# pyg-team/pyg-lib

Hardware: AMD Instinct MI355X
Metric: segment_matmul GFLOP/s + sampled-edges/sec, 1/2/4/8 MI355X vs CPU ref (higher is better)
Workload: dtype bf16; 1 GPU; segment_matmul ogbn-mag-shaped: 154 relations, 21,111,007 rows, F_in=F_out=128 (BASELINE.json configs[1]); relations=154, rows=21111007, rows_per_gpu=21111007, F=128

## Files before the change

### pyg_lib_amd/csrc/hip/matmul_dw.hip

```cpp
#include "matmul_dw_out.h"

#include <stdint.h>

#include <algorithm>
#include <atomic>

namespace pyg_hip {
namespace {

typedef __bf16 bf16x8 __attribute__((ext_vector_type(8)));
typedef _Float16 f16x8 __attribute__((ext_vector_type(8)));
typedef short v4i16 __attribute__((ext_vector_type(4)));
typedef short v8i16 __attribute__((ext_vector_type(8)));
typedef float f32x16 __attribute__((ext_vector_type(16)));
typedef uint32_t u32x4 __attribute__((ext_vector_type(4)));

constexpr int kTile = 128;

struct bf16_tag {};
struct f16_tag {};
template <typename Tag>
struct OutOf;
template <>
struct OutOf<bf16_tag> {
  using type = bf16_t;
};
template <>
struct OutOf<f16_tag> {
  using type = f16_t;
};

__device__ __forceinline__ f32x16 mfma16(bf16_tag, v8i16 a, v8i16 b, f32x16 c) {
  return __builtin_amdgcn_mfma_f32_32x32x16_bf16(__builtin_bit_cast(bf16x8, a), __builtin_bit_cast(bf16x8, b), c, 0, 0, 0);
}
__device__ __forceinline__ f32x16 mfma16(f16_tag, v8i16 a, v8i16 b, f32x16 c) {
  return __builtin_amdgcn_mfma_f32_32x32x16_f16(__builtin_bit_cast(f16x8, a), __builtin_bit_cast(f16x8, b), c, 0, 0, 0);
}

constexpr int pitch_bytes(int cols) {
  const int dw = cols / 2;
  const int extra = dw > 16 ? (dw - 16 + 63) / 64 : 0;
  return (16 + 64 * extra) * 4;
}

typedef const __attribute__((address_space(1))) u32x4 GU32x4;

template <typename Tag, int K, int MC>
__global__ __launch_bounds__(256, 1) void seg_dw_kernel(const DwGroup* __restrict__ groups,
                                                         const int32_t* __restrict__ tile_start, int B, int M,
                                                         float* __restrict__ slabs,
                                                         typename OutOf<Tag>::type* __restrict__ out) {
  constexpr int IB = K / 32, JB = MC / 32;
  constexpr int PX = pitch_bytes(K), PY = pitch_bytes(MC);
  constexpr int CX = K / 8, CY = MC / 8;
  constexpr int NX = 32 * CX / 64, NY = 32 * CY / 64;
  static_assert(IB * JB <= 16, "accumulators must fit the register file");
  extern __shared__ __attribute__((aligned(16))) char smem[];
  const int tid = threadIdx.x, lane = tid & 63, wave = tid >> 6;
  const int swave = __builtin_amdgcn_readfirstlane(wave);
  char* xs = smem + wave * 32 * (PX + PY);
  char* ys = xs + 32 * PX;
  const int ncol = M / MC;
  const int bx = ncol > 1 ? ((int)blockIdx.x / (8 * ncol)) * 8 + ((int)blockIdx.x & 7) : (int)blockIdx.x;
  const int by = ncol > 1 ? ((int)blockIdx.x / 8) % ncol : 0;
  const int col0 = by * MC;

  const int total = tile_start[B];
  const int G = (int)gridDim.x / ncol;
  const int t_beg = (int)((int64_t)bx * total / G);
  const int t_end = (int)((int64_t)(bx + 1) * total / G);
  if (t_beg >= t_end) return;
  int g = 0;
  {
    int lo = 0, hi = B;
    while (hi - lo > 1) {
      const int mid = (lo + hi) >> 1;
      if (tile_start[mid] <= t_beg) lo = mid; else hi = mid;
    }
    g = lo;
  }

  f32x16 acc[IB][JB];
#pragma unroll
  for (int i = 0; i < IB; ++i)
#pragma unroll
    for (int j = 0; j < JB; ++j)
#pragma unroll
      for (int r = 0; r < 16; ++r) acc[i][j][r] = 0.0f;
  int acc_g = -1;

  auto flush = [&]() {
    if (acc_g < 0) return;
    using Pos = DwPosRows<IB, JB>;
    const int u0 = tile_start[acc_g], u1 = tile_start[acc_g + 1];
    const bool head = u0 < t_beg, tail = !head && u1 > t_end;
    float* slab = dw_slab(slabs, (int64_t)IB * JB * kDwBlockFloats, ncol, bx, by, head ? 0 : 1);
    typename OutOf<Tag>::type* base = out + ((int64_t)acc_g * K) * M + col0;
    dw_combine_waves<IB, JB>(acc, smem, swave, lane, [&](int bt, int q, dwf4 s) __attribute__((always_inline)) {
      if (head || tail) dw_quarter_to_slab(slab, bt, q, s, lane);
      else dw_quarter_to_out<Pos>(base, M, K, MC, bt, q, s, lane);
    });
#pragma unroll
    for (int i = 0; i < IB; ++i)
#pragma unroll
      for (int j = 0; j < JB; ++j)
#pragma unroll
        for (int r = 0; r < 16; ++r) acc[i][j][r] = 0.0f;
  };

  u32x4 xr[NX], yr[NY];
  int n_g = g;
  DwGroup gd = groups[g];
  auto prefetch = [&](int t) {
    while (t >= tile_start[n_g + 1]) {
      ++n_g;
      gd = groups[n_g];
    }
    const int64_t row0 = (int64_t)(t - tile_start[n_g]) * kTile + wave * 32;
#pragma unroll
    for (int it = 0; it < NX; ++it) {
      const int p = it * 64 + lane;
      const int64_t row = row0 + p / CX;
      u32x4 v = {0u, 0u, 0u, 0u};
      if (row < gd.rows) v = *(GU32x4*)(gd.x + row * K + (p % CX) * 8);
      xr[it] = v;
    }
#pragma unroll
    for (int it = 0; it < NY; ++it) {
      const int p = it * 64 + lane;
      const int64_t row = row0 + p / CY;
      u32x4 v = {0u, 0u, 0u, 0u};
      if (row < gd.rows) v = *(GU32x4*)(gd.dy + row * M + col0 + (p % CY) * 8);
      yr[it] = v;
    }
  };

  const int q = lane & 15, half = (lane >> 4) & 1, kb = lane >> 5;
  const int a_off = (kb * 8 + (q >> 2)) * PX + (half * 16 + (q & 3) * 4) * 2;
  const int b_off = (kb * 8 + (q >> 2)) * PY + (half * 16 + (q & 3) * 4) * 2;
  typedef __attribute__((address_space(3))) v4i16* lds_v4;

  prefetch(t_beg);
  for (int t = t_beg; t < t_end; ++t) {
    const int cur_g = n_g;
    if (cur_g != acc_g) {
      flush();
      acc_g = cur_g;
    }
#pragma unroll
    for (int it = 0; it < NX; ++it) {
      const int p = it * 64 + lane;
      *reinterpret_cast<u32x4*>(xs + (p / CX) * PX + (p % CX) * 16) = xr[it];
    }
#pragma unroll
    for (int it = 0; it < NY; ++it) {
      const int p = it * 64 + lane;
      *reinterpret_cast<u32x4*>(ys + (p / CY) * PY + (p % CY) * 16) = yr[it];
    }
    __builtin_amdgcn_fence(__ATOMIC_RELEASE, "wavefront");
    __builtin_amdgcn_wave_barrier();
    if (t + 1 < t_end) prefetch(t + 1);
#pragma unroll
    for (int ks = 0; ks < 2; ++ks) {
      v8i16 af[IB], bf[JB];
#pragma unroll
      for (int i = 0; i < IB; ++i) {
        const char* p = xs + a_off + ks * 16 * PX + i * 64;
        const v4i16 lo = __builtin_amdgcn_ds_read_tr16_b64_v4i16((lds_v4)(p));
        const v4i16 hi = __builtin_amdgcn_ds_read_tr16_b64_v4i16((lds_v4)(p + 4 * PX));
        af[i] = __builtin_shufflevector(lo, hi, 0, 1, 2, 3, 4, 5, 6, 7);
      }
#pragma unroll
      for (int j = 0; j < JB; ++j) {
        const char* p = ys + b_off + ks * 16 * PY + j * 64;
        const v4i16 lo = __builtin_amdgcn_ds_read_tr16_b64_v4i16((lds_v4)(p));
        const v4i16 hi = __builtin_amdgcn_ds_read_tr16_b64_v4i16((lds_v4)(p + 4 * PY));
        bf[j] = __builtin_shufflevector(lo, hi, 0, 1, 2, 3, 4, 5, 6, 7);
      }
#pragma unroll
      for (int i = 0; i < IB; ++i)
#pragma unroll
        for (int j = 0; j < JB; ++j) acc[i][j] = mfma16(Tag{}, af[i], bf[j], acc[i][j]);
    }
    __builtin_amdgcn_wave_barrier();
  }
  flush();
}

template <typename Tag>
__global__ __launch_bounds__(256, 1) void seg_dw_wide256_kernel(const DwGroup* __restrict__ groups,
                                                                const int32_t* __restrict__ tile_start, int B, int M,
                                                                float* __restrict__ slabs,
                                                                typename OutOf<Tag>::type* __restrict__ out) {
  constexpr int K = 256, MC = 256, IB = K / 32, JB = 2;
  constexpr int PX = pitch_bytes(K), PY = pitch_bytes(MC);
  constexpr int CX = K / 8, CY = MC / 8;
  constexpr int NX = 32 * CX / 256, NY = 32 * CY / 256;
  constexpr int IMG = 32 * (PX + PY);
  extern __shared__ __attribute__((aligned(16))) char smem[];
  const int tid = threadIdx.x, lane = tid & 63, wave = tid >> 6;
  const int swave = __builtin_amdgcn_readfirstlane(wave);
  const int ncol = M / MC;
  const int bx = ncol > 1 ? ((int)blockIdx.x / (8 * ncol)) * 8 + ((int)blockIdx.x & 7) : (int)blockIdx.x;
  const int by = ncol > 1 ? ((int)blockIdx.x / 8) % ncol : 0;
  const int col0 = by * MC;

  const int total = tile_start[B];
  const int G = (int)gridDim.x / ncol;
  const int t_beg = (int)((int64_t)bx * total / G);
  const int t_end = (int)((int64_t)(bx + 1) * total / G);
  if (t_beg >= t_end) return;
  int g = 0;
  {
    int lo = 0, hi = B;
    while (hi - lo > 1) {
      const int mid = (lo + hi) >> 1;
      if (tile_start[mid] <= t_beg) lo = mid; else hi = mid;
    }
    g = lo;
  }

  f32x16 acc[IB][JB];
#pragma unroll
  for (int i = 0; i < IB; ++i)
#pragma unroll
    for (int j = 0; j < JB; ++j)
#pragma unroll
      for (int r = 0; r < 16; ++r) acc[i][j][r] = 0.0f;
  int acc_g = -1;
  auto flush = [&]() {
    if (acc_g < 0) return;
    const int u0 = tile_start[acc_g], u1 = tile_start[acc_g + 1];
    const bool head = u0 < t_beg, tail = !head && u1 > t_end;
    float* slab = dw_slab(slabs, (int64_t)DwPosWide::kBlocks * kDwBlockFloats, ncol, bx, by, head ? 0 : 1);
    typename OutOf<Tag>::type* base = out + ((int64_t)acc_g * K) * M + col0;
    char* stage = smem + 2 * IMG + wave * 16384 + lane * 16;
#pragma unroll
    for (int Q = 0; Q < 4; ++Q) {
#pragma unroll
      for (int L = 0; L < 4; ++L) {
        const int b = Q * 4 + L;
#pragma unroll
        for (int q = 0; q < 4; ++q) {
          const dwf4 v = {acc[b / JB][b % JB][4 * q], acc[b / JB][b % JB][4 * q + 1], acc[b / JB][b % JB][4 * q + 2],
                          acc[b / JB][b % JB][4 * q + 3]};
          *reinterpret_cast<dwf4*>(stage + (L * 4 + q) * 1024) = v;
        }
      }
      __builtin_amdgcn_fence(__ATOMIC_RELEASE, "wavefront");
      __builtin_amdgcn_wave_barrier();
#pragma unroll 1
      for (int it = 0; it < 16; ++it) {
        const dwf4 v = *reinterpret_cast<const dwf4*>(stage + it * 1024);
        const int bt = swave * 16 + Q * 4 + (it >> 2), q = it & 3;
        if (head || tail) dw_quarter_to_slab(slab, bt, q, v, lane);
        else dw_quarter_to_out<DwPosWide>(base, M, K, MC, bt, q, v, lane);
      }
      __builtin_amdgcn_wave_barrier();
    }
#pragma unroll
    for (int i = 0; i < IB; ++i)
#pragma unroll
      for (int j = 0; j < JB; ++j)
#pragma unroll
        for (int r = 0; r < 16; ++r) acc[i][j][r] = 0.0f;
  };

  const int s_beg = t_beg * 4, s_end = t_end * 4;
  u32x4 xr[NX], yr[NY];
  int n_g = g;
  DwGroup gd = groups[g];
  auto prefetch = [&](int sl) {
    const int t = sl >> 2;
    while (t >= tile_start[n_g + 1]) {
      ++n_g;
      gd = groups[n_g];
    }
    const int64_t row0 = (int64_t)(t - tile_start[n_g]) * kTile + (sl & 3) * 32;
#pragma unroll
    for (int it = 0; it < NX; ++it) {
      const int p = it * 256 + tid;
      const int64_t row = row0 + p / CX;
      u32x4 v = {0u, 0u, 0u, 0u};
      if (row < gd.rows) v = *(GU32x4*)(gd.x + row * K + (p % CX) * 8);
      xr[it] = v;
    }
#pragma unroll
    for (int it = 0; it < NY; ++it) {
      const int p = it * 256 + tid;
      const int64_t row = row0 + p / CY;
      u32x4 v = {0u, 0u, 0u, 0u};
      if (row < gd.rows) v = *(GU32x4*)(gd.dy + row * M + col0 + (p % CY) * 8);
      yr[it] = v;
    }
  };
  auto park = [&](int buf) {
    char* xs = smem + buf * IMG;
    char* ys = xs + 32 * PX;
#pragma unroll
    for (int it = 0; it < NX; ++it) {
      const int p = it * 256 + tid;
      *reinterpret_cast<u32x4*>(xs + (p / CX) * PX + (p % CX) * 16) = xr[it];
    }
#pragma unroll
    for (int it = 0; it < NY; ++it) {
      const int p = it * 256 + tid;
      *reinterpret_cast<u32x4*>(ys + (p / CY) * PY + (p % CY) * 16) = yr[it];
    }
  };

  const int q = lane & 15, half = (lane >> 4) & 1, kb = lane >> 5;
  const int a_off = (kb * 8 + (q >> 2)) * PX + (half * 16 + (q & 3) * 4) * 2;
  const int b_off = (kb * 8 + (q >> 2)) * PY + (half * 16 + (q & 3) * 4) * 2 + wave * 128;
  typedef __attribute__((address_space(3))) v4i16* lds_v4;

  prefetch(s_beg);
  int g_img[2];
  g_img[0] = n_g;
  park(0);
  g_img[1] = n_g;
  if (s_beg + 1 < s_end) prefetch(s_beg + 1);
  int g_regs = n_g;
  __syncthreads();

  for (int sl = s_beg; sl < s_end; ++sl) {
    const int cur = (sl - s_beg) & 1;
    if (sl + 1 < s_end) {
      park(cur ^ 1);
      g_img[cur ^ 1] = g_regs;
      if (sl + 2 < s_end) {
        prefetch(sl + 2);
        g_regs = n_g;
      }
    }
    const int cur_g = g_img[cur];
    if (cur_g != acc_g) {
      flush();
      acc_g = cur_g;
    }
    const char* xs = smem + cur * IMG;
    const char* ys = xs + 32 * PX;
#pragma unroll
    for (int ks = 0; ks < 2; ++ks) {
      v8i16 af[IB], bf[JB];
#pragma unroll
      for (int i = 0; i < IB; ++i) {
        const char* p = xs + a_off + ks * 16 * PX + i * 64;
        const v4i16 lo = __builtin_amdgcn_ds_read_tr16_b64_v4i16((lds_v4)(p));
        const v4i16 hi = __builtin_amdgcn_ds_read_tr16_b64_v4i16((lds_v4)(p + 4 * PX));
        af[i] = __builtin_shufflevector(lo, hi, 0, 1, 2, 3, 4, 5, 6, 7);
      }
#pragma unroll
      for (int j = 0; j < JB; ++j) {
        const char* p = ys + b_off + ks * 16 * PY + j * 64;
        const v4i16 lo = __builtin_amdgcn_ds_read_tr16_b64_v4i16((lds_v4)(p));
        const v4i16 hi = __builtin_amdgcn_ds_read_tr16_b64_v4i16((lds_v4)(p + 4 * PY));
        bf[j] = __builtin_shufflevector(lo, hi, 0, 1, 2, 3, 4, 5, 6, 7);
      }
#pragma unroll
      for (int i = 0; i < IB; ++i)
#pragma unroll
        for (int j = 0; j < JB; ++j) acc[i][j] = mfma16(Tag{}, af[i], bf[j], acc[i][j]);
    }
    __syncthreads();
  }
  flush();
}

template <int K, int MC>
__global__ __launch_bounds__(256, 1) void seg_dw_f32_kernel(const DwGroup* __restrict__ groups,
                                                             const int32_t* __restrict__ tile_start, int B, int M,
                                                             float* __restrict__ slabs, float* __restrict__ out) {
  constexpr int IB = K / 32, JB = MC / 32;
  static_assert(IB * JB <= 16, "accumulators must fit the register file");
  constexpr int VA = IB >= 4 ? 4 : IB, VB = JB >= 4 ? 4 : JB;
  extern __shared__ __attribute__((aligned(16))) char smem[];
  const int tid = threadIdx.x, lane = tid & 63, wave = tid >> 6;
  const int swave = __builtin_amdgcn_readfirstlane(wave);
  const int li = lane & 31, kk = lane >> 5;
  const int ncol = M / MC;
  const int bx = ncol > 1 ? ((int)blockIdx.x / (8 * ncol)) * 8 + ((int)blockIdx.x & 7) : (int)blockIdx.x;
  const int by = ncol > 1 ? ((int)blockIdx.x / 8) % ncol : 0;
  const int col0 = by * MC;
  const int total = tile_start[B];
  const int G = (int)gridDim.x / ncol;
  const int t_beg = (int)((int64_t)bx * total / G);
  const int t_end = (int)((int64_t)(bx + 1) * total / G);
  if (t_beg >= t_end) return;
  int g = 0;
  {
    int lo = 0, hi = B;
    while (hi - lo > 1) {
      const int mid = (lo + hi) >> 1;
      if (tile_start[mid] <= t_beg) lo = mid; else hi = mid;
    }
    g = lo;
  }
  f32x16 acc[IB][JB];
#pragma unroll
  for (int i = 0; i < IB; ++i)
#pragma unroll
    for (int j = 0; j < JB; ++j)
#pragma unroll
      for (int r = 0; r < 16; ++r) acc[i][j][r] = 0.0f;
  int acc_g = -1;
  auto flush = [&]() {
    if (acc_g < 0) return;
    using Pos = DwPosF32<IB, JB>;
    const int u0 = tile_start[acc_g], u1 = tile_start[acc_g + 1];
    const bool head = u0 < t_beg, tail = !head && u1 > t_end;
    float* slab = dw_slab(slabs, (int64_t)IB * JB * kDwBlockFloats, ncol, bx, by, head ? 0 : 1);
    float* base = out + ((int64_t)acc_g * K) * M + col0;
    dw_combine_waves<IB, JB>(acc, smem, swave, lane, [&](int bt, int q, dwf4 s) __attribute__((always_inline)) {
      if (head || tail) dw_quarter_to_slab(slab, bt, q, s, lane);
      else dw_quarter_to_out<Pos>(base, M, K, MC, bt, q, s, lane);
    });
#pragma unroll
    for (int i = 0; i < IB; ++i)
#pragma unroll
      for (int j = 0; j < JB; ++j)
#pragma unroll
        for (int r = 0; r < 16; ++r) acc[i][j][r] = 0.0f;
  };
  constexpr int D = 8;
  const int n_it = (t_end - t_beg) * 16;
  float pa[D][IB], pb[D][JB];
  int pg[D];
  int lg = g;
  DwGroup ld = groups[lg];
  auto request = [&](int it, float (&a)[IB], float (&b)[JB], int& grp) {
    const int t = t_beg + (it >> 4);
    while (t >= tile_start[lg + 1]) {
      ++lg;
      ld = groups[lg];
    }
    grp = lg;
    const float* xp = reinterpret_cast<const float*>(ld.x);
    const float* yp = reinterpret_cast<const float*>(ld.dy);
    const int64_t row = (int64_t)(t - tile_start[lg]) * kTile + wave * 32 + 2 * (it & 15) + kk;
    const bool ok = row < ld.rows;
#pragma unroll
    for (int h = 0; h < IB / VA; ++h) {
      typedef float vecA __attribute__((ext_vector_type(VA)));
      vecA v;
#pragma unroll
      for (int e = 0; e < VA; ++e) v[e] = 0.0f;
      if (ok) v = *(const __attribute__((address_space(1))) vecA*)(xp + row * K + 32 * VA * h + VA * li);
#pragma unroll
      for (int e = 0; e < VA; ++e) a[VA * h + e] = v[e];
    }
#pragma unroll
    for (int h = 0; h < JB / VB; ++h) {
      typedef float vecB __attribute__((ext_vector_type(VB)));
      vecB v;
#pragma unroll
      for (int e = 0; e < VB; ++e) v[e] = 0.0f;
      if (ok) v = *(const __attribute__((address_space(1))) vecB*)(yp + row * M + col0 + 32 * VB * h + VB * li);
#pragma unroll
      for (int e = 0; e < VB; ++e) b[VB * h + e] = v[e];
    }
  };
#pragma unroll
  for (int k = 0; k < D; ++k) request(k, pa[k], pb[k], pg[k]);
  static_assert(16 % D == 0, "a chunk of D steps must stay inside one tile");
  for (int it0 = 0; it0 < n_it; it0 += D) {
    if (pg[0] != acc_g) {
      flush();
      acc_g = pg[0];
    }
#pragma unroll
    for (int k = 0; k < D; ++k) {
#pragma unroll
      for (int i = 0; i < IB; ++i)
#pragma unroll
        for (int j = 0; j < JB; ++j) acc[i][j] = __builtin_amdgcn_mfma_f32_32x32x2f32(pa[k][i], pb[k][j], acc[i][j], 0, 0, 0);
      if (it0 + k + D < n_it) request(it0 + k + D, pa[k], pb[k], pg[k]);
    }
  }
  flush();
}

template <typename Pos, typename OutT>
__global__ __launch_bounds__(256) void seg_dw_fixup_kernel(const int32_t* __restrict__ tile_start, int B, int K, int M, int MC,
                                                          int G, int fix_blocks, const float* __restrict__ slabs,
                                                          OutT* __restrict__ out) {
  constexpr int NBT = Pos::kBlocks;
  const int lane = threadIdx.x & 63, wave = threadIdx.x >> 6;
  if ((int)blockIdx.x >= fix_blocks) {
    const int g = (int)blockIdx.x - fix_blocks;
    if (tile_start[g + 1] != tile_start[g]) return;
    OutT* base = out + (int64_t)g * K * M;
    for (int i = threadIdx.x; i < K * M; i += 256) dw_put(base + i, 0.0f);
    return;
  }
  const int ncol = M / MC;
  const int v = (int)blockIdx.x * 4 + wave;
  const int m = v / (4 * NBT), piece = v - m * (4 * NBT);
  const int bt = piece >> 2, q = piece & 3;
  const int bx = m / ncol, by = m - bx * ncol;
  const int total = tile_start[B];
  const int t_beg = (int)((int64_t)bx * total / G), t_end = (int)((int64_t)(bx + 1) * total / G);
  if (t_beg >= t_end) return;
  int lo = 0, hi = B;
  while (hi - lo > 1) {
    const int mid = (lo + hi) >> 1;
    if (tile_start[mid] <= t_end - 1) lo = mid; else hi = mid;
  }
  const int u0 = tile_start[lo], u1 = tile_start[lo + 1];
  if (!(u1 > t_end && u0 >= t_beg)) return;
  const dwf4 s = dw_chain_sum(slabs, (int64_t)NBT * kDwBlockFloats, ncol, bx, by, G, total, u1, bt, q, lane);
  dw_quarter_to_out<Pos>(out + (int64_t)lo * K * M + by * MC, M, K, MC, bt, q, s, lane);
}

__host__ __device__ inline int64_t dw_describe(DwGroup& d, const char* x, const char* dy, int64_t rows, int64_t, int64_t, int,
                                               int64_t, int, int) {
  d.x = reinterpret_cast<const uint16_t*>(x);
  d.dy = reinterpret_cast<const uint16_t*>(dy);
  d.rows = rows;
  return 1;
}
__host__ __device__ inline int64_t dw_describe(DwGenGroup& d, const char* x, const char* dy, int64_t rows, int64_t k, int64_t m,
                                               int elt, int64_t acc_off, int kb, int mb) {
  auto mn = [](int a, int b) { return a < b ? a : b; };
  d.x = x;
  d.dy = dy;
  d.rows = rows;
  d.acc_off = acc_off;
  d.k = (int32_t)k;
  d.m = (int32_t)m;
  d.lx = (int16_t)mn(gen_log2_align((uint64_t)x), gen_log2_align((uint64_t)(k * elt)));
  d.ly = (int16_t)mn(gen_log2_align((uint64_t)dy), gen_log2_align((uint64_t)(m * elt)));
  d.nkb = (int16_t)((k + kb - 1) / kb);
  d.nmb = (int16_t)((m + mb - 1) / mb);
  return (int64_t)d.nkb * d.nmb;
}

template <typename Desc>
__global__ void dw_plan_kernel(const int64_t* __restrict__ ptr, int64_t B, const char* X, const char* dY, int64_t K, int64_t M,
                               int elt, int kb, int mb, Desc* __restrict__ groups, int32_t* __restrict__ tile_start) {
  __shared__ int64_t part[256];
  const int tid = threadIdx.x;
  const int64_t per = (B + 255) / 256;
  const int64_t beg = min((int64_t)tid * per, B), end = min(beg + per, B);
  Desc d;
  const int64_t blocks = dw_describe(d, X, dY, 0, K, M, elt, 0, kb, mb);
  int64_t t = 0;
  for (int64_t b = beg; b < end; ++b) {
    const int64_t r = ptr[b + 1] - ptr[b];
    t += r > 0 ? (r + kTile - 1) / kTile * blocks : 0;
  }
  part[tid] = t;
  __syncthreads();
  if (tid == 0) {
    int64_t acc = 0;
    for (int i = 0; i < 256; ++i) {
      const int64_t v = part[i];
      part[i] = acc;
      acc += v;
    }
    tile_start[B] = (int32_t)acc;
  }
  __syncthreads();
  t = part[tid];
  for (int64_t b = beg; b < end; ++b) {
    tile_start[b] = (int32_t)t;
    const int64_t p0 = ptr[b];
    const int64_t r = ptr[b + 1] - p0;
    dw_describe(d, X + p0 * K * elt, dY + p0 * M * elt, r > 0 ? r : 0, K, M, elt, b * K * M, kb, mb);
    groups[b] = d;
    t += r > 0 ? (r + kTile - 1) / kTile * blocks : 0;
  }
}

enum class DwFamily {
  kUnsupported,
  kInvalid,
  kGen,
  kSeg,
  kWide256,
};
struct DwRoute {
  DwFamily family;
  int K = 0, MC = 0;
};

inline bool dw_dtype_ok(int dtype) { return dtype == PYG_F32 || dtype == PYG_BF16 || dtype == PYG_F16; }
inline int dw_elt(int dtype) { return dtype == PYG_F32 ? 4 : 2; }
inline DwRoute dw_gen_route(int dtype) { return {DwFamily::kGen, kDwGenKB, dw_gen_mb(dw_elt(dtype))}; }

DwRoute choose_dw_route(int dtype, int64_t K, int64_t M, bool uniform, unsigned misalign) {
  if (!dw_dtype_ok(dtype)) return {DwFamily::kUnsupported};
  if (misalign % dw_elt(dtype) != 0) return {DwFamily::kInvalid};
  if (!uniform || misalign % 16 != 0 || !((K == 64 || K == 128 || K == 256) && M > 0 && M % 64 == 0)) {
    if (K >= (1LL << 21) || M >= (1LL << 21) || K * M >= (1LL << 28)) return {DwFamily::kUnsupported};
    return dw_gen_route(dtype);
  }
  if (dtype != PYG_F32 && K == 256 && M % 256 == 0) return {DwFamily::kWide256, 256, 256};
  return {DwFamily::kSeg, (int)K, K == 256 || M % 128 != 0 ? 64 : 128};
}

inline unsigned dw_misalign(uintptr_t operands, const void* out, int elt) {
  return (unsigned)((operands & 15) | ((uintptr_t)out & (uintptr_t)(elt - 1)));
}

const char* dw_route_name(int dtype, DwRoute r) {
  thread_local char name[32];
  const char* t = dtype == PYG_BF16 ? "bf16" : dtype == PYG_F16 ? "f16" : "f32";
  switch (r.family) {
    case DwFamily::kUnsupported: return "unsupported";
    case DwFamily::kInvalid: return "invalid";
    case DwFamily::kGen: return "gen";
    case DwFamily::kSeg: snprintf(name, sizeof(name), "seg_%s_k%d_mc%d", t, r.K, r.MC); break;
    case DwFamily::kWide256: snprintf(name, sizeof(name), "wide256_%s", t); break;
  }
  return name;
}

int dw_route_check(const char* op, DwRoute r, int64_t K, int64_t M) {
  if (r.family == DwFamily::kInvalid) return fail(PYG_HIP_ERR_INVALID, "%s: operands must be element-aligned", op);
  if (r.family == DwFamily::kUnsupported)
    return fail(PYG_HIP_ERR_UNSUPPORTED, "%s: K x M = %lld x %lld is beyond the kernel's 32-bit offsets", op, (long long)K,
                (long long)M);
  if (r.family == DwFamily::kGen)
    PYG_HIP_REQUIRE((K + r.K - 1) / r.K < 32768 && (M + r.MC - 1) / r.MC < 32768, "%s: K / M too large", op);
  return PYG_HIP_OK;
}

inline int64_t dw_ncol(DwRoute r, int64_t M) { return r.family == DwFamily::kGen ? 1 : M / r.MC; }
inline int64_t dw_grid_x(int64_t tiles_upper, int64_t ncol) {
  int64_t gx = std::max<int64_t>(1, std::min<int64_t>(tiles_upper, device_info().num_cus / ncol));
  if (ncol > 1) gx = (gx + 7) / 8 * 8;
  return gx;
}
inline size_t dw_slab_bytes(DwRoute r, int64_t M) {
  const int64_t ncol = dw_ncol(r, M);
  return (size_t)(dw_grid_x(INT64_MAX, ncol) * ncol) * 2 * (size_t)r.K * (size_t)r.MC * sizeof(float);
}

struct DwWorkspace {
  int64_t* ptr_copy;
  void* descs;
  int32_t* tile_start;
  float* slabs;
  size_t plan_bytes;
  size_t bytes;
};

DwWorkspace carve_dw(void* ws, int64_t B, size_t desc_size, size_t slab_bytes) {
  DwWorkspace w;
  size_t off = 0;
  auto take = [&](size_t bytes, size_t align) {
    void* p = reinterpret_cast<void*>(reinterpret_cast<uintptr_t>(ws) + off);
    off += align_up(bytes, align);
    return p;
  };
  w.ptr_copy = static_cast<int64_t*>(take(sizeof(int64_t) * (size_t)(B + 1), 256));
  w.descs = take(desc_size * (size_t)std::max<int64_t>(B, 1), 256);
  w.tile_start = static_cast<int32_t*>(take(sizeof(int32_t) * (size_t)(B + 1), 256));
  w.plan_bytes = off - (size_t)(static_cast<char*>(w.descs) - static_cast<char*>(ws));
  w.slabs = static_cast<float*>(take(slab_bytes, 1));
  w.bytes = off;
  return w;
}
DwWorkspace carve_dw(void* ws, int64_t B, DwRoute r, int64_t M) {
  return carve_dw(ws, B, r.family == DwFamily::kGen ? sizeof(DwGenGroup) : sizeof(DwGroup), dw_slab_bytes(r, M));
}

size_t dw_workspace_bytes(int64_t B, int64_t K, int64_t M, bool uniform) {
  size_t need = 0;
  for (int dtype : {PYG_BF16, PYG_F32}) {
    need = std::max(need, carve_dw(nullptr, B, dw_gen_route(dtype), M).bytes);
    const DwRoute r = choose_dw_route(dtype, K, M, uniform, 0);
    if (r.family == DwFamily::kSeg || r.family == DwFamily::kWide256) need = std::max(need, carve_dw(nullptr, B, r, M).bytes);
  }
  return need;
}

struct DwLaunch {
  const DwGroup* groups;
  const int32_t* tile_start;
  int64_t B, M;
  int64_t gx;
  float* slabs;
  void* out;
  hipStream_t stream;
};

template <typename Pos, typename OutT>
int launch_fixup(const DwLaunch& a, int K, int MC, OutT* out) {
  const int64_t ncol = a.M / MC;
  const int64_t fix_blocks = a.gx * ncol * Pos::kBlocks;
  hipLaunchKernelGGL((seg_dw_fixup_kernel<Pos, OutT>), dim3((unsigned)(fix_blocks + a.B)), dim3(256), 0, a.stream, a.tile_start,
                     (int)a.B, K, (int)a.M, MC, (int)a.gx, (int)fix_blocks, a.slabs, out);
  PYG_HIP_CHECK(hipGetLastError());
  return PYG_HIP_OK;
}

template <typename Tag, int K, int MC>
int launch_dw(const DwLaunch& a) {
  using OutT = typename OutOf<Tag>::type;
  OutT* out = static_cast<OutT*>(a.out);
  constexpr int lds = 4 * 32 * (pitch_bytes(K) + pitch_bytes(MC));
  static_assert(lds >= (K / 32) * (MC / 32) * 4096, "the combine area must fit the row images");
  const void* kern = reinterpret_cast<const void*>(&seg_dw_kernel<Tag, K, MC>);
  if (int rc_ = ensure_dynamic_lds(kern, lds)) return rc_;
  hipLaunchKernelGGL((seg_dw_kernel<Tag, K, MC>), dim3((unsigned)(a.gx * (a.M / MC))), dim3(256), lds, a.stream, a.groups,
                     a.tile_start, (int)a.B, (int)a.M, a.slabs, out);
  PYG_HIP_CHECK(hipGetLastError());
  return launch_fixup<DwPosRows<K / 32, MC / 32>, OutT>(a, K, MC, out);
}

template <typename Tag>
int launch_dw_wide256(const DwLaunch& a) {
  using OutT = typename OutOf<Tag>::type;
  OutT* out = static_cast<OutT*>(a.out);
  constexpr int lds = 2 * 32 * (pitch_bytes(256) + pitch_bytes(256)) + 4 * 16384;
  const void* kern = reinterpret_cast<const void*>(&seg_dw_wide256_kernel<Tag>);
  if (int rc_ = ensure_dynamic_lds(kern, lds)) return rc_;
  hipLaunchKernelGGL((seg_dw_wide256_kernel<Tag>), dim3((unsigned)(a.gx * (a.M / 256))), dim3(256), lds, a.stream, a.groups,
                     a.tile_start, (int)a.B, (int)a.M, a.slabs, out);
  PYG_HIP_CHECK(hipGetLastError());
  return launch_fixup<DwPosWide, OutT>(a, 256, 256, out);
}

template <int K, int MC>
int launch_dw_f32(const DwLaunch& a) {
  float* out = static_cast<float*>(a.out);
  constexpr int lds = (K / 32) * (MC / 32) * 4096;
  const void* kern = reinterpret_cast<const void*>(&seg_dw_f32_kernel<K, MC>);
  if (int rc_ = ensure_dynamic_lds(kern, lds)) return rc_;
  hipLaunchKernelGGL((seg_dw_f32_kernel<K, MC>), dim3((unsigned)(a.gx * (a.M / MC))), dim3(256), lds, a.stream, a.groups,
                     a.tile_start, (int)a.B, (int)a.M, a.slabs, out);
  PYG_HIP_CHECK(hipGetLastError());
  return launch_fixup<DwPosF32<K / 32, MC / 32>, float>(a, K, MC, out);
}

template <int K, int MC>
int launch_seg(int dtype, const DwLaunch& a) {
  return dtype == PYG_F32 ? launch_dw_f32<K, MC>(a) : dtype == PYG_BF16 ? launch_dw<bf16_tag, K, MC>(a) : launch_dw<f16_tag, K, MC>(a);
}

int run_dw_route(DwRoute r, int dtype, const DwWorkspace& w, int64_t B, int64_t M, int64_t tiles_upper, void* out, int lg,
                 hipStream_t stream) {
  const int64_t gx = dw_grid_x(tiles_upper, dw_ncol(r, M));
  const DwLaunch a = {static_cast<const DwGroup*>(w.descs), w.tile_start, B, M, gx, w.slabs, out, stream};
  switch (r.family) {
    case DwFamily::kGen: return launch_dw_gen(dtype, w.descs, w.tile_start, (int)B, gx, w.slabs, out, lg, stream);
    case DwFamily::kWide256: return dtype == PYG_BF16 ? launch_dw_wide256<bf16_tag>(a) : launch_dw_wide256<f16_tag>(a);
    case DwFamily::kSeg:
      if (r.K == 128 && r.MC == 128) return launch_seg<128, 128>(dtype, a);
      if (r.K == 128 && r.MC == 64) return launch_seg<128, 64>(dtype, a);
      if (r.K == 64 && r.MC == 128) return launch_seg<64, 128>(dtype, a);
      if (r.K == 64 && r.MC == 64) return launch_seg<64, 64>(dtype, a);
      if (r.K == 256 && r.MC == 64) return launch_seg<256, 64>(dtype, a);
      break;
    default: break;
  }
  return fail(PYG_HIP_ERR_INVALID, "matmul_dw: unknown route");
}

std::atomic<int64_t> g_dw_fast{0}, g_dw_gen{0};
inline int dw_count(DwRoute r, int rc) {
  if (rc == PYG_HIP_OK) ++(r.family == DwFamily::kGen ? g_dw_gen : g_dw_fast);
  return rc;
}

template <typename Desc>
int dw_segment(DwRoute r, int dtype, const void* input, const int64_t* ptr, int ptr_on_device, const void* grad_out,
               void* grad_other, int64_t N, int64_t K, int64_t M, int64_t B, void* workspace, hipStream_t stream) {
  const int elt = dw_elt(dtype);
  const char* X = static_cast<const char*>(input);
  const char* dY = static_cast<const char*>(grad_out);
  Desc d;
  const int64_t tiles_upper = ((N + kTile - 1) / kTile + B) * dw_describe(d, X, dY, 0, K, M, elt, 0, r.K, r.MC);
  PYG_HIP_REQUIRE(tiles_upper < (1LL << 31), "segment_matmul_dw: too many tiles");
  const DwWorkspace w = carve_dw(workspace, B, r, M);
  const int64_t* dptr = ptr;
  if (!ptr_on_device) {
    if (int rc = stage_host_ptr("segment_matmul_dw", ptr, B, N, w.ptr_copy, stream)) return rc;
    dptr = w.ptr_copy;
  }
  hipLaunchKernelGGL(dw_plan_kernel<Desc>, dim3(1), dim3(256), 0, stream, dptr, B, X, dY, K, M, elt, r.K, r.MC,
                     static_cast<Desc*>(w.descs), w.tile_start);
  PYG_HIP_CHECK(hipGetLastError());
  const int lg = gen_log2_align((uint64_t)input | (uint64_t)(K * elt) | (uint64_t)grad_out | (uint64_t)(M * elt));
  return run_dw_route(r, dtype, w, B, M, tiles_upper, grad_other, lg, stream);
}

template <typename Desc>
int dw_grouped(DwRoute r, int dtype, const pyg_hip_group* host_groups, int64_t G, void* out_pool, void* workspace,
               hipStream_t stream) {
  const int elt = dw_elt(dtype);
  const DwWorkspace w = carve_dw(workspace, G, r, host_groups[0].m);
  void* staged = nullptr;
  int rc = pinned_stage().acquire(w.plan_bytes, &staged);
  if (rc != PYG_HIP_OK) return rc;
  Desc* hd = static_cast<Desc*>(staged);
  int32_t* ht = reinterpret_cast<int32_t*>(static_cast<char*>(staged) + (reinterpret_cast<char*>(w.tile_start) - static_cast<char*>(w.descs)));
  int64_t t = 0, off = 0;
  int lg = 4;
  for (int64_t i = 0; i < G; ++i) {
    const pyg_hip_group& g = host_groups[i];
    ht[i] = (int32_t)t;
    t += (g.rows + kTile - 1) / kTile * dw_describe(hd[i], static_cast<const char*>(g.input), static_cast<const char*>(g.other),
                                                    g.rows, g.k, g.m, elt, off, r.K, r.MC);
    PYG_HIP_REQUIRE(t < (1LL << 31), "grouped_matmul_dw: too many tiles");
    if (g.rows > 0 && g.k > 0 && g.m > 0)
      lg = std::min(lg, gen_log2_align((uint64_t)g.input | (uint64_t)(g.k * elt) | (uint64_t)g.other | (uint64_t)(g.m * elt)));
    off += (int64_t)g.k * g.m;
  }
  ht[G] = (int32_t)t;
  PYG_HIP_CHECK(hipMemcpyAsync(w.descs, staged, w.plan_bytes, hipMemcpyHostToDevice, stream));
  rc = pinned_stage().commit(stream);
  if (rc != PYG_HIP_OK) return rc;
  if (r.family != DwFamily::kGen) return run_dw_route(r, dtype, w, G, host_groups[0].m, t + 1, out_pool, lg, stream);
  if (off == 0) return PYG_HIP_OK;
  if (t == 0) {
    PYG_HIP_CHECK(hipMemsetAsync(out_pool, 0, (size_t)elt * (size_t)off, stream));
    return PYG_HIP_OK;
  }
  return run_dw_route(r, dtype, w, G, 0, t, out_pool, lg, stream);
}

}
}

using namespace pyg_hip;

extern "C" {

void pyg_hip_matmul_dw_counters(int64_t* specialised, int64_t* general) {
  if (specialised) *specialised = g_dw_fast.load();
  if (general) *general = g_dw_gen.load();
}

const char* pyg_hip_matmul_dw_route(int dtype, int64_t K, int64_t M, int uniform, unsigned misalign) {
  if (K < 0 || M < 0) return "invalid";
  return dw_route_name(dtype, choose_dw_route(dtype, K, M, uniform != 0, misalign));
}

size_t pyg_hip_segment_matmul_dw_workspace_size(int64_t B, int64_t K, int64_t M) {
  return dw_workspace_bytes(std::max<int64_t>(B, 0), std::max<int64_t>(K, 0), std::max<int64_t>(M, 0), true);
}

size_t pyg_hip_grouped_matmul_dw_workspace_size(const pyg_hip_group* groups, int64_t G) {
  if (G <= 0 || groups == nullptr) return dw_workspace_bytes(0, 0, 0, false);
  bool uniform = true;
  for (int64_t i = 0; i < G; ++i) uniform = uniform && groups[i].k == groups[0].k && groups[i].m == groups[0].m;
  return dw_workspace_bytes(G, std::max(groups[0].k, 0), std::max(groups[0].m, 0), uniform);
}

int pyg_hip_segment_matmul_dw(int dtype, const void* input, const int64_t* ptr, int ptr_on_device, const void* grad_out,
                              void* grad_other, int64_t N, int64_t K, int64_t M, int64_t B, void* workspace,
                              size_t workspace_bytes, void* stream_) {
  hipStream_t stream = static_cast<hipStream_t>(stream_);
  PYG_HIP_REQUIRE(N >= 0 && K >= 0 && M >= 0 && B >= 0, "segment_matmul_dw: negative size");
  if (B * K * M == 0) return PYG_HIP_OK;
  PYG_HIP_REQUIRE(ptr && grad_other && (N == 0 || (input && grad_out)), "segment_matmul_dw: NULL tensor");
  if (!dw_dtype_ok(dtype))
    return fail(PYG_HIP_ERR_UNSUPPORTED, "segment_matmul_dw: float32 / bfloat16 / float16 only (dtype %d)", dtype);
  const size_t need = pyg_hip_segment_matmul_dw_workspace_size(B, K, M);
  if (workspace == nullptr || workspace_bytes < need)
    return fail(PYG_HIP_ERR_WORKSPACE, "segment_matmul_dw: workspace of %zu bytes needed, got %zu", need, workspace_bytes);
  const unsigned misalign = dw_misalign((uintptr_t)input | (uintptr_t)grad_out, grad_other, dw_elt(dtype));
  const DwRoute r = choose_dw_route(dtype, K, M, true, misalign);
  if (int rc = dw_route_check("segment_matmul_dw", r, K, M)) return rc;
  return dw_count(r, r.family == DwFamily::kGen
                         ? dw_segment<DwGenGroup>(r, dtype, input, ptr, ptr_on_device, grad_out, grad_other, N, K, M, B, workspace, stream)
                         : dw_segment<DwGroup>(r, dtype, input, ptr, ptr_on_device, grad_out, grad_other, N, K, M, B, workspace, stream));
}

int pyg_hip_grouped_matmul_dw(int dtype, const pyg_hip_group* host_groups, int64_t G, void* out_pool, void* workspace,
                              size_t workspace_bytes, void* stream_) {
  hipStream_t stream = static_cast<hipStream_t>(stream_);
  PYG_HIP_REQUIRE(G >= 0 && G < (1LL << 31), "grouped_matmul_dw: bad group count");
  if (G == 0) return PYG_HIP_OK;
  PYG_HIP_REQUIRE(host_groups && out_pool, "grouped_matmul_dw: NULL argument");
  if (!dw_dtype_ok(dtype))
    return fail(PYG_HIP_ERR_UNSUPPORTED, "grouped_matmul_dw: float32 / bfloat16 / float16 only (dtype %d)", dtype);
  const int64_t K = host_groups[0].k, M = host_groups[0].m;
  bool uniform = true;
  uintptr_t operands = 0;
  for (int64_t i = 0; i < G; ++i) {
    const pyg_hip_group& g = host_groups[i];
    PYG_HIP_REQUIRE(g.rows >= 0 && g.k >= 0 && g.m >= 0, "grouped_matmul_dw: negative size in group %lld", (long long)i);
    PYG_HIP_REQUIRE(g.rows == 0 || g.k == 0 || g.m == 0 || (g.input && g.other), "grouped_matmul_dw: NULL tensor in group %lld",
                    (long long)i);
    uniform = uniform && g.k == K && g.m == M;
    operands |= (uintptr_t)g.input | (uintptr_t)g.other;
  }
  const size_t need = pyg_hip_grouped_matmul_dw_workspace_size(host_groups, G);
  if (workspace == nullptr || workspace_bytes < need)
    return fail(PYG_HIP_ERR_WORKSPACE, "grouped_matmul_dw: workspace of %zu bytes needed, got %zu", need, workspace_bytes);
  const unsigned misalign = dw_misalign(operands, out_pool, dw_elt(dtype));
  const DwRoute r = choose_dw_route(dtype, K, M, uniform, misalign);
  for (int64_t i = 0; i < G; ++i) {
    const int64_t k = host_groups[i].k, m = host_groups[i].m;
    if (int rc = dw_route_check("grouped_matmul_dw", choose_dw_route(dtype, k, m, uniform, misalign), k, m)) return rc;
  }
  return dw_count(r, r.family == DwFamily::kGen ? dw_grouped<DwGenGroup>(r, dtype, host_groups, G, out_pool, workspace, stream)
                                                : dw_grouped<DwGroup>(r, dtype, host_groups, G, out_pool, workspace, stream));
}

}
```

Baseline: 388,600 GFLOP/s.

## Add ring-buffered direct-to-LDS pipeline for 128x128 segment dW kernel

Adds a new dW kernel for K=MC=128 in which each wave keeps a 4-slot LDS ring. The ring is filled with global_load_lds_dwordx4 (direct global-to-LDS, non-temporal) using XOR-swizzled offsets, and vmcnt waits let three items load ahead of the MFMA work. This removes the register staging and the per-tile LDS store/barrier round trip of the old kernel. Partial tail rows go through a separate zero-padded path. The default launch path now routes 128x128 to the new kernel. An experiment macro also adds a load-only probe mode. The hand-written m0 and vmcnt asm is fragile and adds correctness risk.

```diff
diff --git a/pyg_lib_amd/csrc/hip/matmul_dw.hip b/pyg_lib_amd/csrc/hip/matmul_dw.hip
--- a/pyg_lib_amd/csrc/hip/matmul_dw.hip
+++ b/pyg_lib_amd/csrc/hip/matmul_dw.hip
@@ -16,6 +16,10 @@
 typedef uint32_t u32x4 __attribute__((ext_vector_type(4)));
 
 constexpr int kTile = 128;
+
+#ifndef PYG_HIP_DW_EXPERIMENTS
+#define PYG_HIP_DW_EXPERIMENTS 0
+#endif
 
 struct bf16_tag {};
 struct f16_tag {};
@@ -147,6 +151,14 @@
       flush();
       acc_g = cur_g;
     }
+#if PYG_HIP_DW_EXPERIMENTS == 2
+#pragma unroll
+    for (int it = 0; it < NX; ++it) asm volatile("" ::"v"(xr[it]));
+#pragma unroll
+    for (int it = 0; it < NY; ++it) asm volatile("" ::"v"(yr[it]));
+    if (t + 1 < t_end) prefetch(t + 1);
+    continue;
+#endif
 #pragma unroll
     for (int it = 0; it < NX; ++it) {
       const int p = it * 64 + lane;
@@ -183,6 +195,194 @@
         for (int j = 0; j < JB; ++j) acc[i][j] = mfma16(Tag{}, af[i], bf[j], acc[i][j]);
     }
     __builtin_amdgcn_wave_barrier();
+  }
+  flush();
+}
+
+template <typename Tag>
+__global__ __launch_bounds__(256, 1) void seg_dw_ring_kernel(const DwGroup* __restrict__ groups,
+                                                              const int32_t* __restrict__ tile_start, int B, int M,
+                                                              float* __restrict__ slabs,
+                                                              typename OutOf<Tag>::type* __restrict__ out) {
+  constexpr int K = 128, MC = 128, IB = K / 32, JB = MC / 32;
+  constexpr int kItem = 8192, kSlots = 4;
+  extern __shared__ __attribute__((aligned(16))) char smem[];
+  const int tid = threadIdx.x, lane = tid & 63;
+  const int swave = __builtin_amdgcn_readfirstlane(tid >> 6);
+  char* ring = smem + swave * (kSlots * kItem);
+  const int ncol = M / MC;
+  const int bx = ncol > 1 ? ((int)blockIdx.x / (8 * ncol)) * 8 + ((int)blockIdx.x & 7) : (int)blockIdx.x;
+  const int by = ncol > 1 ? ((int)blockIdx.x / 8) % ncol : 0;
+  const int col0 = by * MC;
+
+  const int total = tile_start[B];
+  const int G = (int)gridDim.x / ncol;
+  const int t_beg = (int)((int64_t)bx * total / G);
+  const int t_end = (int)((int64_t)(bx + 1) * total / G);
+  if (t_beg >= t_end) return;
+  int g = 0;
+  {
+    int lo = 0, hi = B;
+    while (hi - lo > 1) {
+      const int mid = (lo + hi) >> 1;
+      if (tile_start[mid] <= t_beg) lo = mid; else hi = mid;
+    }
+    g = lo;
+  }
+
+  f32x16 acc[IB][JB];
+#pragma unroll
+  for (int i = 0; i < IB; ++i)
+#pragma unroll
+    for (int j = 0; j < JB; ++j)
+#pragma unroll
+      for (int r = 0; r < 16; ++r) acc[i][j][r] = 0.0f;
+  int acc_g = -1;
+
+  auto flush = [&]() {
+    if (acc_g < 0) return;
+    using Pos = DwPosRows<IB, JB>;
+    const int u0 = tile_start[acc_g], u1 = tile_start[acc_g + 1];
+    const bool head = u0 < t_beg, tail = !head && u1 > t_end;
+    float* slab = dw_slab(slabs, (int64_t)IB * JB * kDwBlockFloats, ncol, bx, by, head ? 0 : 1);
+    typename OutOf<Tag>::type* base = out + ((int64_t)acc_g * K) * M + col0;
+    dw_combine_waves<IB, JB>(acc, smem, swave, lane, [&](int bt, int q, dwf4 s) __attribute__((always_inline)) {
+      if (head || tail) dw_quarter_to_slab(slab, bt, q, s, lane);
+      else dw_quarter_to_out<Pos>(base, M, K, MC, bt, q, s, lane);
+    });
+    asm volatile("s_waitcnt vmcnt(0)" ::: "memory");
+#pragma unroll
+    for (int i = 0; i < IB; ++i)
+#pragma unroll
+      for (int j = 0; j < JB; ++j)
+#pragma unroll
+        for (int r = 0; r < 16; ++r) acc[i][j][r] = 0.0f;
+  };
+
+  const int l4 = lane >> 4, cs = lane & 15;
+  const uint32_t src_chunk = (uint32_t)((cs ^ (l4 << 2)) * 16);
+  uint32_t ox[4], oy[4];
+#pragma unroll
+  for (int j = 0; j < 4; ++j) {
+    ox[j] = (uint32_t)((4 * j + l4) * (K * 2)) + src_chunk;
+    oy[j] = (uint32_t)(4 * j + l4) * (uint32_t)(M * 2) + (uint32_t)(col0 * 2) + src_chunk;
+  }
+  const int q = lane & 15, half = (lane >> 4) & 1, kb = lane >> 5, rho = q >> 2;
+  int rd[4];
+#pragma unroll
+  for (int i = 0; i < 4; ++i) rd[i] = (kb * 8 + rho) * 256 + ((i ^ rho) * 64) + half * 32 + (q & 3) * 8;
+  typedef __attribute__((address_space(3))) v4i16* lds_v4;
+
+  DwGroup gd = groups[g];
+  const uint32_t ring_lds = (uint32_t)(size_t)ring;
+  auto issue = [&](int64_t row, int slot) {
+    const char* xb = reinterpret_cast<const char*>(gd.x) + row * (K * 2);
+    const char* yb = reinterpret_cast<const char*>(gd.dy) + row * ((int64_t)M * 2);
+    const uint32_t lds = ring_lds + (uint32_t)(slot * kItem);
+    uint32_t sv;
+    asm volatile(
+        "s_waitcnt lgkmcnt(0)\n\t"
+        "s_nop 4\n\t"
+        "s_mov_b32 %[sv], m0\n\t"
+        "s_mov_b32 m0, %[lds]\n\t"
+        "s_nop 0\n\t"
+        "global_load_lds_dwordx4 %[x0], %[xb] nt\n\t"
+        "s_add_u32 m0, m0, 0x400\n\ts_nop 0\n\t"
+        "global_load_lds_dwordx4 %[x1], %[xb] nt\n\t"
+        "s_add_u32 m0, m0, 0x400\n\ts_nop 0\n\t"
+        "global_load_lds_dwordx4 %[x2], %[xb] nt\n\t"
+        "s_add_u32 m0, m0, 0x400\n\ts_nop 0\n\t"
+        "global_load_lds_dwordx4 %[x3], %[xb] nt\n\t"
+        "s_add_u32 m0, m0, 0x400\n\ts_nop 0\n\t"
+        "global_load_lds_dwordx4 %[y0], %[yb] nt\n\t"
+        "s_add_u32 m0, m0, 0x400\n\ts_nop 0\n\t"
+        "global_load_lds_dwordx4 %[y1], %[yb] nt\n\t"
+        "s_add_u32 m0, m0, 0x400\n\ts_nop 0\n\t"
+        "global_load_lds_dwordx4 %[y2], %[yb] nt\n\t"
+        "s_add_u32 m0, m0, 0x400\n\ts_nop 0\n\t"
+        "global_load_lds_dwordx4 %[y3], %[yb] nt\n\t"
+        "s_mov_b32 m0, %[sv]"
+        : [sv] "=&s"(sv)
+        : [lds] "s"(lds), [xb] "s"(xb), [yb] "s"(yb), [x0] "v"(ox[0]), [x1] "v"(ox[1]), [x2] "v"(ox[2]), [x3] "v"(ox[3]),
+          [y0] "v"(oy[0]), [y1] "v"(oy[1]), [y2] "v"(oy[2]), [y3] "v"(oy[3])
+        : "memory", "scc");
+  };
+  auto wait_item = [&](int younger) {
+    if (younger >= 3) asm volatile("s_waitcnt vmcnt(24)" ::: "memory");
+    else if (younger == 2) asm volatile("s_waitcnt vmcnt(16)" ::: "memory");
+    else if (younger == 1) asm volatile("s_waitcnt vmcnt(8)" ::: "memory");
+    else asm volatile("s_waitcnt vmcnt(0)" ::: "memory");
+  };
+  auto multiply = [&](int slot) {
+    const char* xs = ring + slot * kItem;
+    const char* ys = xs + kItem / 2;
+    v8i16 af[IB], bf[JB];
+#pragma unroll
+    for (int i = 0; i < IB; ++i) {
+      const char* p = xs + rd[i];
+      const v4i16 lo = __builtin_amdgcn_ds_read_tr16_b64_v4i16((lds_v4)(p));
+      const v4i16 hi = __builtin_amdgcn_ds_read_tr16_b64_v4i16((lds_v4)(p + 4 * 256));
+      af[i] = __builtin_shufflevector(lo, hi, 0, 1, 2, 3, 4, 5, 6, 7);
+    }
+#pragma unroll
+    for (int j = 0; j < JB; ++j) {
+      const char* p = ys + rd[j];
+      const v4i16 lo = __builtin_amdgcn_ds_read_tr16_b64_v4i16((lds_v4)(p));
+      const v4i16 hi = __builtin_amdgcn_ds_read_tr16_b64_v4i16((lds_v4)(p + 4 * 256));
+      bf[j] = __builtin_shufflevector(lo, hi, 0, 1, 2, 3, 4, 5, 6, 7);
+    }
+#pragma unroll
+    for (int i = 0; i < IB; ++i)
+#pragma unroll
+      for (int j = 0; j < JB; ++j) acc[i][j] = mfma16(Tag{}, af[i], bf[j], acc[i][j]);
+  };
+  auto park_partial = [&](int64_t row, int nrows, int slot) {
+    char* xs = ring + slot * kItem;
+    char* ys = xs + kItem / 2;
+    u32x4 xv[4], yv[4];
+#pragma unroll
+    for (int j = 0; j < 4; ++j) {
+      xv[j] = u32x4{0u, 0u, 0u, 0u};
+      yv[j] = u32x4{0u, 0u, 0u, 0u};
+      if (4 * j + l4 < nrows) {
+        xv[j] = *(GU32x4*)(reinterpret_cast<const char*>(gd.x) + row * (K * 2) + ox[j]);
+        yv[j] = *(GU32x4*)(reinterpret_cast<const char*>(gd.dy) + row * ((int64_t)M * 2) + oy[j]);
+      }
+    }
+#pragma unroll
+    for (int j = 0; j < 4; ++j) {
+      *reinterpret_cast<u32x4*>(xs + j * 1024 + lane * 16) = xv[j];
+      *reinterpret_cast<u32x4*>(ys + j * 1024 + lane * 16) = yv[j];
+    }
+    __builtin_amdgcn_fence(__ATOMIC_RELEASE, "wavefront");
+    __builtin_amdgcn_wave_barrier();
+  };
+
+  for (int t = t_beg; t < t_end;) {
+    while (t >= tile_start[g + 1]) ++g;
+    const int g_end = tile_start[g + 1];
+    const int t1 = g_end < t_end ? g_end : t_end;
+    flush();
+    acc_g = g;
+    gd = groups[g];
+    const int64_t row0 = (int64_t)(t - tile_start[g]) * kTile + swave * 32;
+    const int T = t1 - t;
+    const int64_t left = gd.rows - (row0 + (int64_t)(T - 1) * kTile);
+    const int nf = 2 * (T - 1) + (left >= 32 ? 2 : left >= 16 ? 1 : 0);
+    const int pr = left > 0 && left < 32 ? (int)(left & 15) : 0;
+    auto row_of = [&](int n) { return row0 + (int64_t)(n >> 1) * kTile + (n & 1) * 16; };
+    for (int n = 0; n < kSlots - 1 && n < nf; ++n) issue(row_of(n), n);
+    for (int n = 0; n < nf; ++n) {
+      if (n + kSlots - 1 < nf) issue(row_of(n + kSlots - 1), (n + kSlots - 1) & (kSlots - 1));
+      wait_item(nf - 1 - n);
+      multiply(n & (kSlots - 1));
+    }
+    if (pr) {
+      park_partial(row_of(nf), pr, nf & (kSlots - 1));
+      multiply(nf & (kSlots - 1));
+    }
+    __builtin_amdgcn_wave_barrier();
+    t = t1;
   }
   flush();
 }
@@ -696,18 +896,36 @@
   return PYG_HIP_OK;
 }
 
+template <typename Tag>
+int launch_dw_ring(const DwLaunch& a) {
+  using OutT = typename OutOf<Tag>::type;
+  OutT* out = static_cast<OutT*>(a.out);
+  constexpr int lds = 4 * 4 * 8192;
+  static_assert(lds >= 16 * 4096, "the combine area must fit the rings");
+  const void* kern = reinterpret_cast<const void*>(&seg_dw_ring_kernel<Tag>);
+  if (int rc_ = ensure_dynamic_lds(kern, lds)) return rc_;
+  hipLaunchKernelGGL((seg_dw_ring_kernel<Tag>), dim3((unsigned)(a.gx * (a.M / 128))), dim3(256), lds, a.stream, a.groups,
+                     a.tile_start, (int)a.B, (int)a.M, a.slabs, out);
+  PYG_HIP_CHECK(hipGetLastError());
+  return launch_fixup<DwPosRows<4, 4>, OutT>(a, 128, 128, out);
+}
+
 template <typename Tag, int K, int MC>
 int launch_dw(const DwLaunch& a) {
   using OutT = typename OutOf<Tag>::type;
   OutT* out = static_cast<OutT*>(a.out);
-  constexpr int lds = 4 * 32 * (pitch_bytes(K) + pitch_bytes(MC));
-  static_assert(lds >= (K / 32) * (MC / 32) * 4096, "the combine area must fit the row images");
-  const void* kern = reinterpret_cast<const void*>(&seg_dw_kernel<Tag, K, MC>);
-  if (int rc_ = ensure_dynamic_lds(kern, lds)) return rc_;
-  hipLaunchKernelGGL((seg_dw_kernel<Tag, K, MC>), dim3((unsigned)(a.gx * (a.M / MC))), dim3(256), lds, a.stream, a.groups,
-                     a.tile_start, (int)a.B, (int)a.M, a.slabs, out);
-  PYG_HIP_CHECK(hipGetLastError());
-  return launch_fixup<DwPosRows<K / 32, MC / 32>, OutT>(a, K, MC, out);
+  if constexpr (K == 128 && MC == 128 && PYG_HIP_DW_EXPERIMENTS == 0) {
+    return launch_dw_ring<Tag>(a);
+  } else {
+    constexpr int lds = 4 * 32 * (pitch_bytes(K) + pitch_bytes(MC));
+    static_assert(lds >= (K / 32) * (MC / 32) * 4096, "the combine area must fit the row images");
+    const void* kern = reinterpret_cast<const void*>(&seg_dw_kernel<Tag, K, MC>);
+    if (int rc_ = ensure_dynamic_lds(kern, lds)) return rc_;
+    hipLaunchKernelGGL((seg_dw_kernel<Tag, K, MC>), dim3((unsigned)(a.gx * (a.M / MC))), dim3(256), lds, a.stream, a.groups,
+                       a.tile_start, (int)a.B, (int)a.M, a.slabs, out);
+    PYG_HIP_CHECK(hipGetLastError());
+    return launch_fixup<DwPosRows<K / 32, MC / 32>, OutT>(a, K, MC, out);
+  }
 }
 
 template <typename Tag>
```

Measured after the change: 389,900 GFLOP/s (median of 5 runs). About the same (+0.3%).
